# ishine/TTS-3

Measured on AMD Instinct MI355X. Metric: audio samples/sec + RTF, HiFiGAN-v1 22.05kHz 80-mel, batch 32 @ 1/2/4/8 GPU, higher is better.
Workload: dtype fp32 (power-of-2 scaled fp16 hi/lo split on fp16 MFMA, fp32 accumulate); 1 GPU; HiFiGAN-v1 22.05kHz inference, [32,80,1024] mel per GPU (replicate pad 5), fp32; model=HiFiGAN-v1 (hifigan_config.py generator_model_params), global_batch=32, seq_len=1024, parallelism=dp1 (utterance sharding; no collectives)

## Files before the change

tts-3_amd/csrc/common.hpp:

```cpp
#pragma once

#include <hip/hip_runtime.h>

#include <cstdint>
#include <stdexcept>
#include <string>

namespace tts {

struct Error : std::runtime_error {
  int code;
  Error(int c, const std::string& m) : std::runtime_error(m), code(c) {}
};

#define TTS_HIP_CHECK(expr)                                                               \
  do {                                                                                    \
    hipError_t _e = (expr);                                                               \
    if (_e != hipSuccess)                                                                 \
      throw ::tts::Error(2, std::string(#expr) + " failed: " + hipGetErrorString(_e));    \
  } while (0)

#define TTS_REQUIRE(cond, code, msg)                    \
  do {                                                  \
    if (!(cond)) throw ::tts::Error((code), (msg));     \
// ... 32 lines not shown
  int mask_res;
  int wn_rows;
  int gate;
  int planes;
};

constexpr int kSplitGateTile = 20;
constexpr int kSplitWinoTile = 21;
bool wino_supported(int mode, int Cout, int Cin, int K, int dil);
bool wino_enabled();
void launch_wino(int mode, const Conv1dArgs& a, int B, int K, hipStream_t s);
inline int gate_row_order(int rho, int H) {
  const int j = rho / 128, r = rho % 128;
  return r < 64 ? 64 * j + r : H + 64 * j + (r - 64);
}

struct ResPairArgs {
  Conv1dArgs c1;
  Conv1dArgs c2;
  const float* post_w;
  float post_bias;
  float post_slope;
  float* wav;
};
bool resblock_pair_supported(int mode, int C, int K, int dil);
bool resblock_pair_preferred(int mode, int C, int K, int dil);
bool resblock_pair128(int mode, int C, int K);
void launch_resblock_pair(int mode, const ResPairArgs& a, int B, int K, int C, int wide64, hipStream_t s);

struct ResBlock3Args {
  const float* x;
  const unsigned* amax_in;
  const float* w[6];
  const float* bias[6];
  int w_exp[6];
  int dil[3];
  float* z;
  int zmode;
  float zdiv;
  unsigned* amax_out;
  int T;
  int planes;
  const float* up_w;
  const float* up_bias;
  int up_w_exp;
  float* up_y;
  unsigned* up_amax;
  const float* zp[2];
  int nzp;
};
bool resblock3_supported(int mode, int C, int K, const int* dil);
bool resblock3_up_supported(int mode, int C, int K, const int* dil, int wide64);
constexpr int kWide64Block = 1, kWide64Pair = 2;
void launch_resblock3(int mode, const ResBlock3Args& a, int B, int C, int K, int wide64, hipStream_t s);
int mrf_geo64_wide(int mode);
bool resblock2_supported(int mode, int C, int K, const int* dil);
bool resblock2_preferred(int mode, int C, int K, const int* dil);
int resblock2_geo64(int mode);
void launch_resblock2(int mode, const ResBlock3Args& a, int B, int C, int K, int geo64, hipStream_t s);

struct ConvTile {
  int BM, BN, TM, TN, CK;
  int PD = 1;
  int WINO = 0;
};

struct ConvTArgs {
  const float* x;
  const float* w;
  const float* bias;
  float* y;
  int Cin, Cout, Tin;
  int n_chunks;
  float in_slope;
  unsigned* amax_out;
  const float* cvec;
};

struct PostArgs {
  const float* z;
  const float* w;
  float bias;
  float* y;
  int Cin, T;
  float in_slope;
  int z_b16;
};

int conv1d_tile_for(int Cout, int K, int Cin, int dil, bool res);
ConvTile conv1d_tile(int idx);
int conv1d_num_tiles();
void launch_conv1d(const Conv1dArgs& a, int B, int K, int tile_idx, hipStream_t s);
int convT_tile_for(int Cout, int U);
ConvTile convT_tile(int idx, int U);
void launch_convT(const ConvTArgs& a, int B, int U, int tile_idx, hipStream_t s);
void launch_conv_post(const PostArgs& a, int B, hipStream_t s);
void launch_mel_window(const float* mel, int B, int C, int T, int pad, int64_t w0, int W, float* out, hipStream_t s);
void launch_cond_vec(const float* g, const float* Wc, const float* bc, float* cvec, int B, int Cc,
                     int C0, hipStream_t s);

constexpr int MATH_FP32 = 0;
constexpr int MATH_FP32_X6 = 1;
constexpr int MATH_FP32_F16X3 = 2;
constexpr int MATH_BF16 = 3;
constexpr int MATH_LAST = MATH_BF16;

ConvTile conv1d_split_tile(int mode, int idx);
int conv1d_split_num_tiles(int mode);
// ... 45 lines not shown
```

tts-3_amd/csrc/hifigan.cpp:

```cpp
#include "hifigan.hpp"

#include <algorithm>
#include <cmath>
#include <cstdlib>
#include <vector>

namespace tts {

namespace {
bool valid_conv_k(int k) { return k == 1 || k == 3 || k == 5 || k == 7 || k == 11; }
}

std::vector<int64_t> hifigan_weight_shapes(const TtsHifiganCfg& c) {
  std::vector<int64_t> n;
  const int C0 = c.upsample_initial_channel;
  n.push_back((int64_t)C0 * c.in_channels * 7);
  n.push_back(C0);
  for (int i = 0; i < c.num_upsamples; ++i) {
    const int ci = C0 >> i, co = C0 >> (i + 1);
    n.push_back((int64_t)ci * co * c.upsample_kernel_sizes[i]);
    n.push_back(co);
  }
  for (int i = 0; i < c.num_upsamples; ++i) {
    const int ch = C0 >> (i + 1);
// ... 27 lines not shown
  TTS_REQUIRE(c.out_channels == 1, 3, "only out_channels == 1 is implemented");
  TTS_REQUIRE(c.resblock_type == 1 || c.resblock_type == 2, 1, "resblock_type must be '1' or '2'");
  TTS_REQUIRE(c.num_kernels >= 1 && c.num_kernels <= TTS_MAX_KERNELS, 1, "bad num_kernels");
  TTS_REQUIRE(c.num_upsamples >= 1 && c.num_upsamples <= TTS_MAX_UPSAMPLES, 1, "bad num_upsamples");
  const int need_d = c.resblock_type == 1 ? 3 : 2;
  TTS_REQUIRE(c.num_dilations >= need_d && c.num_dilations <= TTS_MAX_DILATIONS, 1,
              "resblock_dilation_sizes too short for the resblock type");
  for (int j = 0; j < c.num_kernels; ++j) {
    TTS_REQUIRE(valid_conv_k(c.resblock_kernel_sizes[j]), 3,
                "resblock kernel size " + std::to_string(c.resblock_kernel_sizes[j]) +
                    " not implemented (1,3,5,7,11)");
    for (int m = 0; m < need_d; ++m) {
      const int d = c.resblock_dilation_sizes[j][m];
      TTS_REQUIRE(d >= 1 && (c.resblock_kernel_sizes[j] - 1) * d <= 96, 3,
                  "resblock (kernel_size-1)*dilation must be <= 96");
    }
  }
  int C = c.upsample_initial_channel;
  for (int i = 0; i < c.num_upsamples; ++i) {
    const int u = c.upsample_factors[i];
    TTS_REQUIRE(u == 2 || u == 4 || u == 8, 3, "upsample factor must be 2, 4 or 8");
    TTS_REQUIRE(c.upsample_kernel_sizes[i] == 2 * u, 3,
                "upsample kernel size must equal 2*factor (polyphase kernel)");
    C >>= 1;
    TTS_REQUIRE(C >= 1, 1, "upsample_initial_channel too small for the number of upsamples");
  }
  TTS_REQUIRE(c.inference_padding >= 0, 1, "inference_padding must be >= 0");
  TTS_REQUIRE(c.cond_channels >= 0, 1, "cond_channels must be >= 0");
  TTS_REQUIRE(!c.cond_in_each_up_layer || c.cond_channels > 0, 1, "cond_in_each_up_layer needs cond_channels > 0");
  TTS_REQUIRE(c.math_mode >= MATH_FP32 && c.math_mode <= MATH_LAST, 1, "unknown math_mode");
}

Hifigan::Hifigan(const TtsHifiganCfg& cfg, const float* const* hw, int device)
    : cfg_(cfg), device_(device) {
  hifigan_validate(cfg_);
  DeviceGuard g(device_);
  const auto shapes = hifigan_weight_shapes(cfg_);
  for (size_t i = 0; i < shapes.size(); ++i)
    TTS_REQUIRE(hw[i] != nullptr, 1, "weight pointer " + std::to_string(i) + " is NULL");

  const int C0 = cfg_.upsample_initial_channel;
  const int mode = cfg_.math_mode;
  const char* nf = std::getenv("TTS_MI355X_NO_PAIR_FUSION");
  const bool pair_fusion = !(nf && nf[0] == '1');
  const char* pf = std::getenv("TTS_MI355X_POST_FUSION");
  post_fusion_ = !(pf && pf[0] == '0');
  const char* ms = std::getenv("TTS_MI355X_MRF_STREAMS");
  nbs_ = ms ? std::max(1, std::min(std::atoi(ms), cfg.num_kernels)) : cfg.num_kernels;
  nbs_env_ = ms != nullptr;
  const char* sb = std::getenv("TTS_MI355X_SUBBATCH");
  n_lanes_ = sb ? std::max(1, std::min(std::atoi(sb), 8)) : 2;
  rb2_geo64_ = resblock2_geo64(mode);
  geo64_wide_ = mrf_geo64_wide(mode);
  const char* bp = std::getenv("TTS_MI355X_BF16_PLANES");
  planes16_ = mode == MATH_BF16 && !(bp && bp[0] == '0') && cfg_.num_upsamples >= 1 &&
              cfg_.upsample_factors[0] % 8 == 0;
  size_t wi = 0;
  std::vector<std::pair<const float*, const float*>> src;
  auto add_conv = [&](int Cin, int Cout, int K, int dil, const char* fam, bool res, int lmode, bool pair128 = false) {
    ConvLayer L;
    L.Cin = Cin; L.Cout = Cout; L.K = K; L.dil = dil; L.pad = dil * (K - 1) / 2;
    L.mode = lmode;
    L.tile = conv_tile_for(lmode, Cout, K, Cin, dil, res);
    if (pair128) {
      L.tile = 7;
      L.name = std::string(fam) + "_k" + std::to_string(K) + "_c" + std::to_string(Cout);
      return L;
    }
    const bool wino_k3 = [] {
      const char* e = std::getenv("TTS_MI355X_WINO_K3");
      return e && e[0] == '1';
    }();
    const bool k_ok = K >= 7 || (K == 3 && Cout >= 256 && wino_k3);
    if (std::string(fam) == "mrf_conv" && k_ok && wino_enabled() && wino_supported(lmode, Cout, Cin, K, dil)) {
      L.tile = kSplitWinoTile;
      fam = "mrf_wino";
    }
    L.name = std::string(fam) + "_k" + std::to_string(K) + "_c" + std::to_string(Cout);
    return L;
  };

  pre_ = add_conv(cfg_.in_channels, C0, 7, 1, "conv_pre", false, mode);
  src.push_back({hw[wi], hw[wi + 1]}); wi += 2;
  for (int i = 0; i < cfg_.num_upsamples; ++i) {
    ConvTLayer L;
    L.Cin = C0 >> i; L.Cout = C0 >> (i + 1); L.U = cfg_.upsample_factors[i];
    L.mode = mode;
    L.tile = is_split_mode(mode) ? conv_tile_for(mode, L.U * L.Cout, 2, L.Cin, 1, false) : convT_tile_for(L.Cout, L.U);
    L.name = "ups_u" + std::to_string(L.U) + "_c" + std::to_string(L.Cout);
    ups_.push_back(L);
  }
  std::vector<std::pair<const float*, const float*>> usrc;
  for (int i = 0; i < cfg_.num_upsamples; ++i) { usrc.push_back({hw[wi], hw[wi + 1]}); wi += 2; }

  for (int i = 0; i < cfg_.num_upsamples; ++i) {
    const int ch = C0 >> (i + 1);
    for (int j = 0; j < cfg_.num_kernels; ++j) {
      const int k = cfg_.resblock_kernel_sizes[j];
      ResBlock rb;
      if (cfg_.resblock_type == 1) {
        const float* w1[3]; const float* b1[3]; const float* w2[3]; const float* b2[3];
        for (int m = 0; m < 3; ++m) { w1[m] = hw[wi]; b1[m] = hw[wi + 1]; wi += 2; }
        for (int m = 0; m < 3; ++m) { w2[m] = hw[wi]; b2[m] = hw[wi + 1]; wi += 2; }
        rb.fused = pair_fusion;
        const bool p128 = pair_fusion && resblock_pair128(mode, ch, k);
        bool tiles_ok = true;
        for (int m = 0; m < 3; ++m) {
          rb.convs.push_back(add_conv(ch, ch, k, cfg_.resblock_dilation_sizes[j][m], "mrf_conv", false, mode, p128));
          src.push_back({w1[m], b1[m]});
          rb.convs.push_back(add_conv(ch, ch, k, 1, "mrf_conv", true, mode, p128));
          src.push_back({w2[m], b2[m]});
          for (int c = 0; c < 2; ++c) {
            const ConvTile t = conv_tile(mode, rb.convs[2 * m + c].tile);
            const int dil = rb.convs[2 * m].dil;
            tiles_ok = tiles_ok && !t.WINO && t.CK % 16 == 0 && ch % t.CK == 0 && ch % t.BM == 0;
            rb.fused = rb.fused && !t.WINO && t.CK == 16 && ceil_div(ch, t.BM) * t.BM == ch &&
                       resblock_pair_preferred(mode, ch, k, dil);
          }
        }
        rb.fused3 = pair_fusion && tiles_ok;
      } else {
        bool tiles_ok = true;
        for (int m = 0; m < 2; ++m) {
          rb.convs.push_back(add_conv(ch, ch, k, cfg_.resblock_dilation_sizes[j][m], "mrf_conv", true, mode));
          src.push_back({hw[wi], hw[wi + 1]}); wi += 2;
          const ConvTile t = conv_tile(mode, rb.convs[m].tile);
          tiles_ok = tiles_ok && !t.WINO && t.CK % 16 == 0 && ch % t.CK == 0 && ch % t.BM == 0;
        }
        rb.fused2 = pair_fusion && tiles_ok;
      }
      if (rb.fused2 || (cfg_.resblock_type == 1 && rb.fused3)) {
        const int policy = [] {
          const char* e = std::getenv("TTS_MI355X_RESBLOCK3");
          if (!e) return 1 << 30;
          if (std::string(e) == "all") return 1 << 30;
          return std::atoi(e);
        }();
        const std::string wk = [] {
          const char* e = std::getenv("TTS_MI355X_RB1_WHOLE_K");
          return std::string(e ? e : "");
        }();
        const bool k_ok = k == 3 || wk.find(std::to_string(k)) != std::string::npos;
        if (cfg_.resblock_type == 1)
          rb.fused3 = ch <= policy && k_ok && resblock3_supported(mode, ch, k, cfg_.resblock_dilation_sizes[j]);
        else
          rb.fused2 = ch <= policy && resblock2_preferred(mode, ch, k, cfg_.resblock_dilation_sizes[j]);
      }
      res_.push_back(rb);
    }
  }
  ups_fused_.assign(cfg_.num_upsamples, 0);
  const char* uf = std::getenv("TTS_MI355X_UPS_FUSION");
  if (!(uf && uf[0] == '0') && cfg_.resblock_type == 1 && cfg_.num_kernels <= 3 && !cfg_.cond_in_each_up_layer &&
      !planes16_) {
    for (int i = 0; i + 1 < cfg_.num_upsamples; ++i) {
      const int ch = C0 >> (i + 1);
      const ConvTLayer& u = ups_[i + 1];
      if (!res_[i * cfg_.num_kernels].fused3 || u.U != 2 || !is_split_mode(u.mode)) continue;
      const ConvTile t = conv_tile(u.mode, u.tile);
      const bool tile_ok = !t.WINO && t.CK % 16 == 0 && ch % t.CK == 0 && ch % t.BM == 0;
      ups_fused_[i] = tile_ok && resblock3_up_supported(mode, ch, cfg_.resblock_kernel_sizes[0],
                                                        cfg_.resblock_dilation_sizes[0], geo64_wide_);
    }
  }
  const float* post_w = hw[wi]; wi += 1;
  post_bias_ = cfg_.conv_post_bias ? hw[wi][0] : 0.f;
  if (cfg_.conv_post_bias) wi += 1;

  HostArena arena;
  std::vector<ConvLayer*> convs;
  convs.push_back(&pre_);
  for (auto& rb : res_) for (auto& c : rb.convs) convs.push_back(&c);
  for (size_t i = 0; i < convs.size(); ++i) {
    ConvLayer& c = *convs[i];
    arena.put_conv(c, c.mode, conv_tile(c.mode, c.tile), src[i].first, src[i].second);
  }
  for (size_t i = 0; i < ups_.size(); ++i) {
    auto& u = ups_[i];
    if (is_split_mode(u.mode)) {
      const ConvTile t = conv_tile(u.mode, u.tile);
      u.n_chunks = ceil_div(u.Cin, t.CK);
      const size_t o = arena.alloc(packed_conv_numel(u.mode, u.U * u.Cout, u.Cin, 2, t), &u.w);
      u.w_exp = pack_convT_split(u.mode, usrc[i].first, u.Cin, u.Cout, u.U, t, arena.at(o));
      std::vector<float> bias((size_t)u.U * u.Cout);
      for (int co = 0; co < u.Cout; ++co)
        for (int ph = 0; ph < u.U; ++ph) bias[(size_t)co * u.U + ph] = usrc[i].second[co];
      arena.put_bias(bias.data(), u.U * u.Cout, t, &u.b);
    } else {
      const ConvTile t = convT_tile(u.tile, u.U);
      u.n_chunks = ceil_div(u.Cin, t.CK);
      const size_t o = arena.alloc(packed_convT_numel(u.Cin, u.Cout, u.U, t), &u.w);
      pack_convT(usrc[i].first, u.Cin, u.Cout, u.U, t, arena.at(o));
      arena.put_bias(usrc[i].second, u.Cout, t, &u.b);
    }
  }
// ... 333 lines not shown
      const hipStream_t sj = bj > 0 ? lane->branch[bj - 1] : s;
      float* bufX = ws + (2 + 2 * bj) * plane;
      float* bufT = bj == 0 ? bufT0 : bufX + plane;
      if (bj > 0) TTS_HIP_CHECK(hipStreamWaitEvent(sj, lane->ev_ups, 0));
      float* const xres = (fuse && j + 1 < K && (conc ? bstream(j + 1) : 0) == bj) ? bufZ : bufX;
      rplane[j] = xres;
      auto zorder = [&] {
        if (!fuse && bj > 0 && bstream(j - 1) != bj) TTS_HIP_CHECK(hipStreamWaitEvent(sj, lane->ev_z[j - 1], 0));
      };
      auto zdone = [&] {
        if (conc) TTS_HIP_CHECK(hipEventRecord(lane->ev_z[j], sj));
      };
      const int zlast = fuse ? 0 : ((cfg_.num_kernels == 1 || j == 0) ? 1 : (j == cfg_.num_kernels - 1 ? 3 : 2));
      const int gj = g0 + 1 + j * 6;
      const int gz = g0 + 1 + cfg_.num_kernels * 6;
      if (fuse && j == 0) {
        const ConvTLayer& Un = ups_[i + 1];
        ResBlock3Args ra{};
        ra.x = bufO; ra.amax_in = slots(g0);
        for (int c = 0; c < 6; ++c) { ra.w[c] = rb.convs[c].w; ra.bias[c] = rb.convs[c].b; ra.w_exp[c] = rb.convs[c].w_exp; }
        for (int m = 0; m < 3; ++m) ra.dil[m] = rb.convs[2 * m].dil;
        ra.zdiv = (float)K;
        ra.T = len;
        ra.nzp = K - 1;
        for (int p = 1; p < K; ++p) {
          ra.zp[p - 1] = rplane[p];
          if (conc && bstream(p) > 0) TTS_HIP_CHECK(hipStreamWaitEvent(s, lane->ev_z[p], 0));
        }
        ra.up_w = Un.w; ra.up_bias = Un.b; ra.up_w_exp = Un.w_exp;
        ra.up_y = bufT0; ra.up_amax = slots(stage_group(i + 1));
        const ConvLayer& L1 = rb.convs[0];
        const double flops = 12.0 * B * L1.Cout * (double)L1.Cin * L1.K * len +
                             2.0 * B * Un.Cout * (double)Un.Cin * 2 * (2.0 * len);
        const double bytes = 4.0 * B * L1.Cout * (double)len * (K + 1) + 4.0 * 6.0 * L1.Cout * L1.Cin * L1.K +
                             4.0 * Un.Cin * Un.Cout * 2 * Un.U;
        const std::string nm = "mrf_block_k" + std::to_string(L1.K) + "_c" + std::to_string(L1.Cout);
        run(prof, s, nm.c_str(), flops, bytes, [&] { launch_resblock3(L1.mode, ra, B, L1.Cout, L1.K, geo64_wide_, s); });
        std::swap(bufO, bufT0);
      } else if (cfg_.resblock_type == 1 && rb.fused3) {
        ResBlock3Args ra{};
        ra.x = bufO; ra.amax_in = slots(g0);
        ra.planes = planes16_ ? kPlaneXB16 | kPlaneYB16 : 0;
        for (int c = 0; c < 6; ++c) { ra.w[c] = rb.convs[c].w; ra.bias[c] = rb.convs[c].b; ra.w_exp[c] = rb.convs[c].w_exp; }
        for (int m = 0; m < 3; ++m) ra.dil[m] = rb.convs[2 * m].dil;
        ra.z = fuse ? xres : bufZ; ra.zmode = fuse ? 1 : zlast; ra.zdiv = (float)cfg_.num_kernels;
        ra.amax_out = !fuse && j == cfg_.num_kernels - 1 ? slots(gz) : nullptr;
        ra.T = len;
        const ConvLayer& L1 = rb.convs[0];
        const double flops = 12.0 * B * L1.Cout * (double)L1.Cin * L1.K * len;
        const double bytes = (planes16_ ? 2.0 : 4.0) * B * L1.Cout * len * (zlast >= 2 ? 3 : 2) +
                             4.0 * 6.0 * L1.Cout * L1.Cin * L1.K;
        const std::string nm = "mrf_block_k" + std::to_string(L1.K) + "_c" + std::to_string(L1.Cout);
        zorder();
        run(prof, sj, nm.c_str(), flops, bytes, [&] { launch_resblock3(L1.mode, ra, B, L1.Cout, L1.K, geo64_wide_, sj); });
        zdone();
      } else if (cfg_.resblock_type == 1 && rb.fused) {
        for (int m = 0; m < 3; ++m) {
          const ConvLayer& L1 = rb.convs[2 * m];
          const ConvLayer& L2 = rb.convs[2 * m + 1];
          const float* xin = (m == 0) ? bufO : (m == 1 ? bufX : bufT);
          const bool last = (m == 2);
          float* xout = (m == 1) ? bufT : (last ? xres : bufX);
          ResPairArgs pa{};
          Conv1dArgs& c1 = pa.c1;
          c1.x = xin; c1.w = L1.w; c1.bias = L1.b; c1.Cin = L1.Cin; c1.Cout = L1.Cout; c1.Tin = len; c1.Tout = len;
          c1.dil = L1.dil; c1.pad = L1.pad; c1.n_chunks = L1.n_chunks; c1.in_slope = 0.1f; c1.out_slope = 0.1f;
          c1.zdiv = 1.f; c1.w_exp = L1.w_exp;
          c1.planes = planes16_ ? kPlaneXB16 | kPlaneYB16 : 0;
          c1.amax_in = (m == 0) ? slots(g0) : slots(gj + 2 * m - 1);
          Conv1dArgs& c2 = pa.c2;
          c2.x = nullptr; c2.w = L2.w; c2.bias = L2.b; c2.res = xin; c2.y = xout; c2.z = bufZ;
          c2.Cin = L2.Cin; c2.Cout = L2.Cout; c2.Tin = len; c2.Tout = len; c2.dil = 1; c2.pad = L2.pad;
          c2.n_chunks = L2.n_chunks; c2.in_slope = 1.f; c2.out_slope = 1.f; c2.zmode = last ? zlast : 0;
          c2.zdiv = (float)cfg_.num_kernels; c2.w_exp = L2.w_exp;
          c2.planes = c1.planes;
          c2.amax_out = last ? (!fuse && j == cfg_.num_kernels - 1 ? slots(gz) : nullptr) : slots(gj + 2 * m + 1);
          const bool post = last && zlast == 3 && i == cfg_.num_upsamples - 1 && post_fusion_ &&
                            cfg_.out_channels == 1;
          if (post) {
            pa.post_w = post_wd_; pa.post_bias = post_bias_; pa.post_slope = 0.01f; pa.wav = wav;
            c2.amax_out = nullptr;
            post_done = true;
          }
          double flops = 4.0 * B * L1.Cout * (double)L1.Cin * L1.K * len;
          const double es = planes16_ ? 2.0 : 4.0;
          double bytes = es * B * L1.Cout * len * (last ? (zlast >= 2 ? 4 : 3) : 3) + 4.0 * 2.0 * L1.Cout * L1.Cin * L1.K;
          if (post) {
            flops += 2.0 * B * len * (double)L1.Cout * 7;
            bytes += 4.0 * B * len - es * B * L1.Cout * len;
          }
          const std::string nm = std::string(post ? "mrf_pair_post_k" : "mrf_pair_k") + std::to_string(L1.K) +
                                 "_c" + std::to_string(L1.Cout);
          if (last) zorder();
          run(prof, sj, nm.c_str(), flops, bytes, [&] { launch_resblock_pair(L1.mode, pa, B, L1.K, L1.Cout, geo64_wide_, sj); });
          if (last) zdone();
        }
      } else if (cfg_.resblock_type == 1) {
        for (int m = 0; m < 3; ++m) {
          const float* xin = (m == 0) ? bufO : bufX;
          const unsigned* xin_amax = (m == 0) ? slots(g0) : slots(gj + 2 * m - 1);
          const bool last = (m == 2);
          conv(rb.convs[2 * m], xin, len, len, 0, 0.1f, 0.1f, nullptr, bufT, 0, nullptr, xin_amax, slots(gj + 2 * m),
               sj);
          if (last) zorder();
          conv(rb.convs[2 * m + 1], bufT, len, len, 0, 1.f, 1.f, xin, last ? xres : bufX, last ? zlast : 0, nullptr,
               slots(gj + 2 * m), last ? (!fuse && j == cfg_.num_kernels - 1 ? slots(gz) : nullptr) : slots(gj + 2 * m + 1), sj);
          if (last) zdone();
// ... 47 lines not shown
```

tts-3_amd/csrc/hifigan.hpp:

```cpp
#pragma once

#include <string>
#include <vector>

#include "arena.hpp"
#include "common.hpp"
#include "tts_mi355x.h"

namespace tts {

struct Profiler {
  struct Rec {
    std::string name;
    double flops, bytes;
    hipEvent_t a, b;
  };
  std::vector<Rec> recs;
  ~Profiler() {
    for (auto& r : recs) {
      (void)hipEventDestroy(r.a);
      (void)hipEventDestroy(r.b);
    }
  }
};
// ... 28 lines not shown
  void reserve(int B, int T, int pad);
  void forward(const float* mel, int B, int C, int T, int pad, const float* g, float* wav,
               hipStream_t s, Profiler* prof);
  int device() const { return device_; }
  int window_halo() const;
  int64_t max_window_frames() const;
  int64_t window_payload() const;

 private:
  struct ConvLayer : PackedConv {
    int mode = 0;
    std::string name;
  };
  struct ConvTLayer : PackedConv {
    int U = 0;
    int mode = 0;
    std::string name;
  };
  struct ResBlock {
    std::vector<ConvLayer> convs;
    bool fused = false;
    bool fused3 = false;
    bool fused2 = false;
  };

  struct Lane {
    hipStream_t own = nullptr;
    std::vector<hipStream_t> branch;
    hipEvent_t ev_ups = nullptr, ev_done = nullptr;
    std::vector<hipEvent_t> ev_z;
    int nbs = 1;
  };
  void forward_plain(const float* mel, int B, int C, int T, int pad, const float* g, float* wav, hipStream_t s,
                     Profiler* prof, float* ws, Lane* lane);
  void ensure_lanes();
  int64_t lane_bytes(int B, int64_t L, int nbs) const;
  int lane_batch(int B, int i) const { return B / n_lanes_ + (i < B % n_lanes_ ? 1 : 0); }
  bool windowed(int64_t L) const;
  int64_t plain_workspace_bytes(int B, int64_t L, bool window) const;
  int64_t window_buffer_bytes(int B, int64_t W) const;
  void reserve_plain(int B, int64_t L, bool window = false);
  int64_t plane_floats(int B, int T, int pad) const;
  int64_t cond_floats(int B) const;
  int amax_groups() const;
  int stage_group(int i) const;
  int n_planes(int nbs) const;
  int split_nbs() const;

  TtsHifiganCfg cfg_;
  int device_;
  int hop_ = 1;
  int rb2_geo64_ = 0;
  int geo64_wide_ = 0;
  bool post_fusion_ = true;
  bool planes16_ = false;
  std::vector<char> ups_fused_;
  int nbs_ = 1;
  int n_lanes_ = 2;
  bool nbs_env_ = false;
  std::vector<Lane> lanes_;
  hipEvent_t ev_start_ = nullptr;
  ConvLayer pre_;
  std::vector<ConvTLayer> ups_;
  std::vector<ResBlock> res_;
  float post_bias_ = 0.f;
  float* post_wd_ = nullptr;
  float* cond_wd_ = nullptr;
  float* cond_bd_ = nullptr;
  std::vector<std::pair<float*, float*>> up_cond_;
  DeviceBuffer arena_, ws_;
  DeviceBuffer win_;
};

}
```

tts-3_amd/csrc/kernels_resblock.hip:

```cpp
#include <algorithm>
#include <cstdlib>
#include <type_traits>

#include "resblock_block.hpp"
#include "split_device.hpp"

namespace tts {




constexpr int kPostK = 7;
constexpr int kPostHalo = 3;

template <class S, int K, int C, int PD, int GEO, bool ALLX = false, bool POST = false, bool SWZ = false>
struct PairCfg {
  static_assert(!SWZ || (GEO == 0 && C == 64 && S::NP == 2 && ALLX), "SWZ: GEO 0 at 64 channels, two-piece rows");
  using ROWS = Res3Rows<S::NP, SWZ>;
  static constexpr int PITCH = ROWS::PITCH;
  static_assert(SWZ || PITCH == S::ROWB, "the padded layout is the scheme's own row");
  static constexpr int RP_W = (GEO == 0 || GEO == 4 || GEO == 5 || GEO == 7) ? 256 : (GEO == 1 ? 192 : 128);
  static constexpr int LEAD = (K - 1) / 2;
  static constexpr int RP_BN = RP_W - 2 * LEAD;
  static constexpr int NW = GEO >= 5 ? 8 : 4;
// ... 461 lines not shown
  const char* e256 = std::getenv("TTS_MI355X_PAIR256");
  if (C == 128) return (K == 7 || K == 11) && !(e128 && e128[0] == '0');
  if (C == 256) {
    const char* e11 = std::getenv("TTS_MI355X_PAIR256_K11");
    return (K == 3 || K == 7 || (K == 11 && e11 && e11[0] == '1')) && !(e256 && e256[0] == '0');
  }
  return false;
}

bool resblock_pair_preferred(int mode, int C, int K, int dil) {
  return resblock_pair_supported(mode, C, K, dil);
}

void launch_resblock_pair(int mode, const ResPairArgs& a, int B, int K, int C, int wide64, hipStream_t s) {
  TTS_REQUIRE(resblock_pair_supported(mode, C, K, a.c1.dil), 3, "resblock pair: unsupported configuration");
  TTS_REQUIRE(a.c1.Cin == C && a.c1.Cout == C && a.c2.Cin == C && a.c2.Cout == C && a.c1.Tin == a.c1.Tout &&
                  a.c2.Tout == a.c1.Tout && a.c1.rep_pad == 0 && a.c2.dil == 1,
              1, "resblock pair: bad arguments");
  TTS_REQUIRE(a.c2.res != a.c2.y || a.c2.zmode != 0, 1, "resblock pair: x and x' must not alias");
  TTS_REQUIRE(a.c1.cvec == nullptr && a.c2.cvec == nullptr && a.c1.bias && a.c2.bias, 1,
              "resblock pair: biases required, no cond vector (both are staged in LDS)");
  TTS_REQUIRE((int64_t)C * a.c1.Tout * 4 < (int64_t(1) << 31), 3, "resblock pair: plane exceeds 2 GiB");
  TTS_REQUIRE(!a.post_w || (a.c2.zmode == 3 && a.c2.res && a.c2.z && a.wav && !a.c2.mask), 1,
              "resblock pair: the fused conv_post needs the final MRF sum (zmode 3) with a residual");
  if (mode == MATH_FP32_F16X3) launch_pair_s<SchemeH3>(a, B, K, C, wide64, s);
  else if (mode == MATH_BF16) launch_pair_s<SchemeB1>(a, B, K, C, 0, s);
  else launch_pair_s<SchemeX6>(a, B, K, C, 0, s);
  TTS_HIP_CHECK(hipGetLastError());
}


namespace {
template <class S, int C, int GEO, int K>
void launch_res3_t(const ResBlock3Args& a, int B, hipStream_t s) {
  using P = Res3Cfg<S, C, GEO, K, 6, r3_xoff(K), r3_lead(K)>;
  dim3 grid(ceil_div(a.T, P::RP_BN), 1, B);
  launch_block_pl<S, C, GEO, K, 6, r3_xoff(K), r3_lead(K)>(a, grid, P::NT, s);
}
template <class S, int C, int GEO>
void launch_res3_up_t(const ResBlock3Args& a, int B, hipStream_t s) {
  using P = Res3Cfg<S, C, GEO, 3, 6, r3_xoff(3), r3_lead(3), true>;
  dim3 grid(ceil_div(a.T, P::RP_BN), 1, B);
  hipLaunchKernelGGL((resblock3_kernel<S, C, GEO, 3, 6, r3_xoff(3), r3_lead(3), 0, true>), grid, dim3(P::NT), 0, s, a);
}
template <class S, bool UP>
void launch_res3_wide64(const ResBlock3Args& a, int B, hipStream_t s) {
  using P = Res3Cfg<S, 64, 0, 3, 6, r3_xoff(3), r3_lead(3), UP, true>;
  static_assert(P::RP_BN == 232, "kept columns [12, 244)");
  dim3 grid(ceil_div(a.T, P::RP_BN), 1, B);
  hipLaunchKernelGGL((resblock3_kernel<S, 64, 0, 3, 6, r3_xoff(3), r3_lead(3), 0, UP, true>), grid, dim3(P::NT), 0, s, a);
}
template <class S>
void launch_res3_s(const ResBlock3Args& a, int B, int C, int K, int wide64, hipStream_t s) {
  if (K == 7) {
    if (C == 32) launch_res3_t<S, 32, 0, 7>(a, B, s);
    else launch_res3_t<S, 64, 0, 7>(a, B, s);
    return;
  }
  if (K == 11) {
    if (C == 32) launch_res3_t<S, 32, 0, 11>(a, B, s);
    else launch_res3_t<S, 64, 0, 11>(a, B, s);
    return;
  }
  if constexpr (std::is_same<S, SchemeH3>::value) {
    if (C == 64 && (wide64 & kWide64Block) && a.planes == 0) {
      launch_res3_wide64<S, false>(a, B, s);
      return;
    }
  }
  if (C == 32) launch_res3_t<S, 32, 0, 3>(a, B, s);
  else if (C == 128) {
    if constexpr (S::NP == 2) launch_res3_t<S, 128, 4, 3>(a, B, s);
    else if constexpr (S::ROWB <= 80) launch_res3_t<S, 128, 3, 3>(a, B, s);
    else throw Error(3, "resblock3: 128 channels need a split scheme of at most 80-byte rows");
  } else launch_res3_t<S, 64, 2, 3>(a, B, s);
}
}

bool resblock3_supported(int mode, int C, int K, const int* dil) {
  if (!is_split_mode(mode)) return false;
  if (K == 3) {
    if (!(C == 32 || C == 64 || (C == 128 && mode != MATH_FP32_X6))) return false;
  } else if (K == 7 || K == 11) {
    if (!(C == 32 || C == 64)) return false;
  } else {
    return false;
  }
  const int hk = (K - 1) / 2;
  int lo = -r3_xoff(K);
  for (int m = 0; m < 3; ++m) {
    if (dil[m] < 1 || hk * dil[m] > r3_xoff(K)) return false;
    lo = std::max(lo + hk * dil[m], 0) + hk;
  }
  return lo <= r3_lead(K);
}

int mrf_geo64_wide(int mode) {
  if (mode != MATH_FP32_F16X3) return 0;
  const char* e = std::getenv("TTS_MI355X_GEO64_WIDE");
  return e && e[0] == '0' ? 0 : (kWide64Block | kWide64Pair);
}

bool resblock3_up_supported(int mode, int C, int K, const int* dil, int wide64) {
  if (mode != MATH_FP32_F16X3 || K != 3 || !(C == 64 || C == 128) || !resblock3_supported(mode, C, K, dil)) return false;
  const int rp_w = C == 64 && (wide64 & kWide64Block) ? 256 : 128;
  int lo = -r3_xoff(K), hi = rp_w + r3_xoff(K);
  for (int m = 0; m < 3; ++m) {
    lo = std::max(lo + dil[m], 0) + 1;
    hi = std::min(hi - dil[m], rp_w) - 1;
  }
  return lo <= r3_lead(K) - 1 && hi >= rp_w - r3_lead(K) + 1;
}

void launch_resblock3(int mode, const ResBlock3Args& a, int B, int C, int K, int wide64, hipStream_t s) {
  TTS_REQUIRE(resblock3_supported(mode, C, K, a.dil), 3, "resblock3: unsupported configuration");
  TTS_REQUIRE((int64_t)C * a.T * 4 < (int64_t(1) << 31), 3, "resblock3: plane exceeds 2 GiB");
  if (a.up_w) {
    TTS_REQUIRE(resblock3_up_supported(mode, C, K, a.dil, wide64), 3, "resblock3: no upsampling tail for this configuration");
    TTS_REQUIRE(a.x && a.up_y && a.up_y != a.x && a.up_bias && a.planes == 0 && a.nzp >= 0 && a.nzp <= 2, 1,
                "resblock3: bad arguments of the upsampling tail");
    for (int p = 0; p < a.nzp; ++p)
      TTS_REQUIRE(a.zp[p] && a.zp[p] != a.up_y, 1, "resblock3: a branch plane is missing or aliases the tail's output");
    if (C == 128) launch_res3_up_t<SchemeH3, 128, 4>(a, B, s);
    else if (wide64 & kWide64Block) launch_res3_wide64<SchemeH3, true>(a, B, s);
    else launch_res3_up_t<SchemeH3, 64, 2>(a, B, s);
    TTS_HIP_CHECK(hipGetLastError());
    return;
  }
  TTS_REQUIRE(a.zmode >= 1 && a.zmode <= 3 && a.z && a.x && a.x != a.z, 1, "resblock3: bad arguments");
  if (mode == MATH_FP32_F16X3) launch_res3_s<SchemeH3>(a, B, C, K, wide64, s);
  else if (mode == MATH_BF16) launch_res3_s<SchemeB1>(a, B, C, K, 0, s);
  else launch_res3_s<SchemeX6>(a, B, C, K, 0, s);
  TTS_HIP_CHECK(hipGetLastError());
}

bool resblock2_supported(int mode, int C, int K, const int* dil) {
  if (!is_split_mode(mode) || !(K == 3 || K == 5 || K == 7 || K == 11)) return false;
  if (!(C == 32 || C == 64 || (C == 128 && mode != MATH_FP32_X6 && (K == 3 || K == 5)))) return false;
  const int H = rb2_halo(K), hk = (K - 1) / 2;
  int lo = -H;
  for (int m = 0; m < 2; ++m) {
    if (dil[m] < 1 || hk * dil[m] > H) return false;
    lo = std::max(lo + hk * dil[m], 0);
  }
  return lo <= H;
}

bool resblock2_preferred(int mode, int C, int K, const int* dil) {
  if (!resblock2_supported(mode, C, K, dil)) return false;
  const char* e = std::getenv("TTS_MI355X_RB2_ALL");
  if (e && e[0] == '1') return true;
  return mode == MATH_BF16 || !(C == 64 && K == 11);
}
// ... 19 lines not shown
```

tts-3_amd/csrc/resblock_block.hpp:

```cpp
#pragma once
#include <type_traits>

#include "res3_layout.hpp"
#include "split_device.hpp"

#ifndef RES_PD_B1
#define RES_PD_B1 2
#endif
#ifndef RES_STAGE_8R
#define RES_STAGE_8R 1
#endif

namespace tts {

#ifndef R3_XR_POL
#define R3_XR_POL 0
#endif
constexpr int R3_XOFF = 5;
constexpr int R3_LEAD = 12;
constexpr int r3_xoff(int K) { return R3_XOFF * ((K - 1) / 2); }
constexpr int r3_lead(int K) { return R3_LEAD * ((K - 1) / 2); }
constexpr int rb2_halo(int K) { return K == 3 ? 4 : (K == 5 ? 12 : (K == 7 ? 9 : 15)); }

template <class S, int C, int GEO, int K = 3, int NCV = 6, int XO = R3_XOFF, int LEAD = R3_LEAD, bool UP = false,
          bool SW = false>
struct Res3Cfg {
  static_assert(!SW || (GEO == 0 && S::NP == 2), "SW: GEO 0's tile, two-piece rows");
  static constexpr bool SWZ = (GEO == 4 || SW) && S::NP == 2;
  static constexpr bool W64 = GEO == 4 || SW;
  static constexpr int RP_W = GEO == 0 ? 256 : (GEO == 1 ? 192 : 128);
  static constexpr int RP_BN = RP_W - 2 * LEAD;
  static constexpr int NW = GEO == 3 ? 8 : 4;
  static constexpr int NT = 64 * NW;
  static constexpr int WN = GEO == 0 ? 4 : 2;
  static constexpr int WM = NW / WN;
  static constexpr int TM = C / 32 / WM;
  static constexpr int TN = RP_W / 32 / WN;
  static constexpr int NC = C / 16;
  static constexpr int PR = RP_W + 2 * XO;
  using ROWS = Res3Rows<S::NP, SWZ>;
  static_assert(SWZ || ROWS::PITCH == S::ROWB, "the padded layout is the scheme's own row");
  static constexpr int LDSB = NC * PR * ROWS::PITCH;
  static constexpr int LDS_TOTAL = LDSB + 2 * NW * 4 + (NCV + UP) * C * 4;
  static_assert(!W64 || LDS_TOTAL <= 80 * 1024, "GEO 4 / SW: two workgroups per CU");
  static_assert(TM >= 1 && TM * WM * 32 == C && TN * WN * 32 == RP_W, "geometry");
};

#ifndef RB3_W_B1
#define RB3_W_B1 0
#endif
#ifndef RB3_W64
#define RB3_W64 2
#endif
template <class S, int C, int GEO, int K, int NCV, int XO, int LEAD, int PL = 0, bool UP = false, bool SW = false>
__global__ __launch_bounds__((Res3Cfg<S, C, GEO, K, NCV, XO, LEAD>::NT))
__attribute__((amdgpu_waves_per_eu(S::NP == 1 && RB3_W_B1 > 0 ? RB3_W_B1
                                                                : (C == 64 && GEO == 2 ? RB3_W64 : (C == 32 || GEO >= 3 || SW ? 2 : 1)))))
void resblock3_kernel(ResBlock3Args a) {
  constexpr bool XB = (PL & kPlaneXB16) != 0, YB = (PL & kPlaneYB16) != 0;
  using PX = PlaneT<XB>;
  using PY = PlaneT<YB>;
  using P = Res3Cfg<S, C, GEO, K, NCV, XO, LEAD, UP, SW>;
  using ROWS = typename P::ROWS;
  static_assert(NCV == 6 || NCV == 2, "ResBlock1 (6 convs) or ResBlock2 (2 convs)");
  static_assert(!UP || (NCV == 6 && S::SCALED && PL == 0), "the upsampling tail: ResBlock1, f16x3, fp32 planes");
  constexpr int NP = S::NP;
  constexpr bool H3 = S::SCALED;
  constexpr int TM = P::TM, TN = P::TN, NC = P::NC, PR = P::PR, RP_W = P::RP_W;
  constexpr int PD = S::NP == 1 ? RES_PD_B1 : 2;
  __shared__ __attribute__((aligned(16))) unsigned char smem[P::LDSB];
  constexpr int NT = P::NT;
  __shared__ float red[2][P::NW];
  __shared__ float bsm[(NCV + UP) * C];

  const int tid = threadIdx.x;
  const int lane = tid & 63;
  const int wave = tid >> 6;
  const int half = lane >> 5;
  const int l32 = lane & 31;
  const int wm = __builtin_amdgcn_readfirstlane(wave / P::WN);
  const int wn = wave % P::WN;
  const int mrow0 = wm * TM * 32;
  const int t0 = blockIdx.x * P::RP_BN;
  const int b = blockIdx.z;
  const int T = a.T;
  const int tx0 = t0 - LEAD;
  const int xcol0 = wn * TN * 32 + l32;
  const unsigned avoff = (unsigned)lane * 16u;
  const unsigned chb = (unsigned)T * PX::ES;
  const rsrc_t rx = make_rsrc(plane_at<XB>(a.x, (size_t)b * C * T), (unsigned)C * chb);
  auto ldx = [&](unsigned off, auto pol_tag, unsigned soff = 0u) -> float {
    if constexpr (XB) return PX::ld(rx, off, soff);
    else return bload_x<decltype(pol_tag)::value>(rx, off, soff);
  };
  constexpr bool SOFF = P::W64;

  int ex = H3 ? amax_exp(a.amax_in, b) : 0;
  f32x16 xr[TM][TN];
// ... 493 lines not shown
```

Measured before the change: 171.4 million samples/s.

## Add wide 512-column GEO 5 tile for 32-channel fused ResBlock1 with K=7/11

Adds a new Res3Cfg geometry (GEO 5) for 32-channel ResBlock1: 512-column tiles, 4 waves laid out along time, swizzled two-piece LDS rows, sized so two workgroups fit per CU. It also enables the whole-block fused path for the K=7 resblock at 32 channels, which previously ran unfused unless an env var listed K=7. The wider tile cuts halo recompute per kept column and the fusion cuts global traffic between convs, at the cost of more LDS per workgroup and possibly fewer blocks in flight. A host-side test replays LDS addressing to check for bank conflicts.

```diff
diff --git a/tts-3_amd/csrc/common.hpp b/tts-3_amd/csrc/common.hpp
--- a/tts-3_amd/csrc/common.hpp
+++ b/tts-3_amd/csrc/common.hpp
@@ -108,8 +108,10 @@
 bool resblock3_supported(int mode, int C, int K, const int* dil);
 bool resblock3_up_supported(int mode, int C, int K, const int* dil, int wide64);
 constexpr int kWide64Block = 1, kWide64Pair = 2;
+constexpr int kWide32Block = 4;
 void launch_resblock3(int mode, const ResBlock3Args& a, int B, int C, int K, int wide64, hipStream_t s);
 int mrf_geo64_wide(int mode);
+int mrf_geo32_wide(int mode);
 bool resblock2_supported(int mode, int C, int K, const int* dil);
 bool resblock2_preferred(int mode, int C, int K, const int* dil);
 int resblock2_geo64(int mode);
diff --git a/tts-3_amd/csrc/hifigan.cpp b/tts-3_amd/csrc/hifigan.cpp
--- a/tts-3_amd/csrc/hifigan.cpp
+++ b/tts-3_amd/csrc/hifigan.cpp
@@ -103,6 +103,7 @@
   n_lanes_ = sb ? std::max(1, std::min(std::atoi(sb), 8)) : 2;
   rb2_geo64_ = resblock2_geo64(mode);
   geo64_wide_ = mrf_geo64_wide(mode);
+  geo32_wide_ = mrf_geo32_wide(mode);
   const char* bp = std::getenv("TTS_MI355X_BF16_PLANES");
   planes16_ = mode == MATH_BF16 && !(bp && bp[0] == '0') && cfg_.num_upsamples >= 1 &&
               cfg_.upsample_factors[0] % 8 == 0;
@@ -191,7 +192,8 @@
           const char* e = std::getenv("TTS_MI355X_RB1_WHOLE_K");
           return std::string(e ? e : "");
         }();
-        const bool k_ok = k == 3 || wk.find(std::to_string(k)) != std::string::npos;
+        const bool k7_block = k == 7 && ch == 32 && (geo32_wide_ & kWide32Block) != 0 && j + 1 < cfg_.num_kernels;
+        const bool k_ok = k == 3 || k7_block || wk.find(std::to_string(k)) != std::string::npos;
         if (cfg_.resblock_type == 1)
           rb.fused3 = ch <= policy && k_ok && resblock3_supported(mode, ch, k, cfg_.resblock_dilation_sizes[j]);
         else
@@ -631,7 +633,8 @@
                              4.0 * 6.0 * L1.Cout * L1.Cin * L1.K;
         const std::string nm = "mrf_block_k" + std::to_string(L1.K) + "_c" + std::to_string(L1.Cout);
         zorder();
-        run(prof, sj, nm.c_str(), flops, bytes, [&] { launch_resblock3(L1.mode, ra, B, L1.Cout, L1.K, geo64_wide_, sj); });
+        run(prof, sj, nm.c_str(), flops, bytes,
+            [&] { launch_resblock3(L1.mode, ra, B, L1.Cout, L1.K, geo64_wide_ | geo32_wide_, sj); });
         zdone();
       } else if (cfg_.resblock_type == 1 && rb.fused) {
         for (int m = 0; m < 3; ++m) {
diff --git a/tts-3_amd/csrc/hifigan.hpp b/tts-3_amd/csrc/hifigan.hpp
--- a/tts-3_amd/csrc/hifigan.hpp
+++ b/tts-3_amd/csrc/hifigan.hpp
@@ -104,6 +104,7 @@
   int hop_ = 1;
   int rb2_geo64_ = 0;
   int geo64_wide_ = 0;
+  int geo32_wide_ = 0;
   bool post_fusion_ = true;
   bool planes16_ = false;
   std::vector<char> ups_fused_;
diff --git a/tts-3_amd/csrc/kernels_resblock.hip b/tts-3_amd/csrc/kernels_resblock.hip
--- a/tts-3_amd/csrc/kernels_resblock.hip
+++ b/tts-3_amd/csrc/kernels_resblock.hip
@@ -537,6 +537,13 @@
 }
 template <class S>
 void launch_res3_s(const ResBlock3Args& a, int B, int C, int K, int wide64, hipStream_t s) {
+  if constexpr (std::is_same<S, SchemeH3>::value) {
+    if (C == 32 && (K == 7 || K == 11) && (wide64 & kWide32Block) && a.planes == 0) {
+      if (K == 7) launch_res3_t<S, 32, 5, 7>(a, B, s);
+      else launch_res3_t<S, 32, 5, 11>(a, B, s);
+      return;
+    }
+  }
   if (K == 7) {
     if (C == 32) launch_res3_t<S, 32, 0, 7>(a, B, s);
     else launch_res3_t<S, 64, 0, 7>(a, B, s);
@@ -584,6 +591,12 @@
   if (mode != MATH_FP32_F16X3) return 0;
   const char* e = std::getenv("TTS_MI355X_GEO64_WIDE");
   return e && e[0] == '0' ? 0 : (kWide64Block | kWide64Pair);
+}
+
+int mrf_geo32_wide(int mode) {
+  if (mode != MATH_FP32_F16X3) return 0;
+  const char* e = std::getenv("TTS_MI355X_GEO32_WIDE");
+  return e && e[0] == '0' ? 0 : kWide32Block;
 }
 
 bool resblock3_up_supported(int mode, int C, int K, const int* dil, int wide64) {
diff --git a/tts-3_amd/csrc/resblock_block.hpp b/tts-3_amd/csrc/resblock_block.hpp
--- a/tts-3_amd/csrc/resblock_block.hpp
+++ b/tts-3_amd/csrc/resblock_block.hpp
@@ -44,6 +44,28 @@
   static constexpr int LDS_TOTAL = LDSB + 2 * NW * 4 + (NCV + UP) * C * 4;
   static_assert(!W64 || LDS_TOTAL <= 80 * 1024, "GEO 4 / SW: two workgroups per CU");
   static_assert(TM >= 1 && TM * WM * 32 == C && TN * WN * 32 == RP_W, "geometry");
+};
+
+template <class S, int C, int K, int NCV, int XO, int LEAD, bool UP, bool SW>
+struct Res3Cfg<S, C, 5, K, NCV, XO, LEAD, UP, SW> {
+  static_assert(C == 32 && S::NP == 2 && NCV == 6 && !UP && !SW, "GEO 5: the 32-channel ResBlock1, two-piece rows");
+  static constexpr bool SWZ = true;
+  static constexpr bool W64 = true;
+  static constexpr int RP_W = 512;
+  static constexpr int RP_BN = RP_W - 2 * LEAD;
+  static constexpr int NW = 4;
+  static constexpr int NT = 64 * NW;
+  static constexpr int WN = 4;
+  static constexpr int WM = 1;
+  static constexpr int TM = 1;
+  static constexpr int TN = RP_W / 32 / WN;
+  static constexpr int NC = C / 16;
+  static constexpr int PR = RP_W + 2 * XO;
+  using ROWS = Res3Rows<S::NP, SWZ>;
+  static constexpr int LDSB = NC * PR * ROWS::PITCH;
+  static constexpr int LDS_TOTAL = LDSB + 2 * NW * 4 + NCV * C * 4;
+  static_assert(LDS_TOTAL <= 80 * 1024, "GEO 5: two workgroups per CU");
+  static_assert(RP_BN > 0 && TN * WN * 32 == RP_W, "geometry");
 };
 
 #ifndef RB3_W_B1
diff --git a/tts-3_amd/tests_native/geo32_layout_check.cpp b/tts-3_amd/tests_native/geo32_layout_check.cpp
--- /dev/null
+++ b/tts-3_amd/tests_native/geo32_layout_check.cpp
@@ -0,0 +1,178 @@
+#include <algorithm>
+#include <cstdio>
+#include <vector>
+
+#include "common.hpp"
+#include "res3_layout.hpp"
+
+using namespace tts;
+
+static int failures = 0;
+#define CHECK(cond, ...)                          \
+  do {                                            \
+    if (!(cond)) {                                \
+      if (failures < 20) {                        \
+        std::fprintf(stderr, "FAIL: " __VA_ARGS__); \
+        std::fprintf(stderr, "\n");               \
+      }                                           \
+      ++failures;                                 \
+    }                                             \
+  } while (0)
+
+using R = Res3Rows<2, true>;
+constexpr int NP = 2, NC = 2, RP_W = 512, NT = 256, TN = 4, C = 32, NCV = 6, PITCH = R::PITCH;
+static long n_reads = 0, n_stores = 0;
+
+static int worst(const std::vector<int>& addr, const std::vector<int>& lanes, int dw, int banks) {
+  std::vector<std::vector<int>> on(banks);
+  for (int l : lanes) {
+    if (addr[l] < 0) continue;
+    for (int j = 0; j < dw; ++j) {
+      const int d = addr[l] / 4 + j;
+      auto& v = on[d % banks];
+      if (std::find(v.begin(), v.end(), d) == v.end()) v.push_back(d);
+    }
+  }
+  size_t w = 0;
+  for (const auto& v : on) w = std::max(w, v.size());
+  return (int)w;
+}
+
+static std::vector<std::vector<int>> read128_groups() {
+  const int a[2][16] = {{0, 1, 2, 3, 12, 13, 14, 15, 20, 21, 22, 23, 24, 25, 26, 27},
+                        {4, 5, 6, 7, 8, 9, 10, 11, 16, 17, 18, 19, 28, 29, 30, 31}};
+  std::vector<std::vector<int>> g;
+  for (int h = 0; h < 2; ++h)
+    for (int s = 0; s < 2; ++s) {
+      std::vector<int> v;
+      for (int i = 0; i < 16; ++i) v.push_back(a[s][i] + 32 * h);
+      g.push_back(v);
+    }
+  return g;
+}
+static std::vector<std::vector<int>> contiguous_groups(int n) {
+  std::vector<std::vector<int>> g;
+  for (int l0 = 0; l0 < 64; l0 += n) {
+    std::vector<int> v;
+    for (int i = 0; i < n; ++i) v.push_back(l0 + i);
+    g.push_back(v);
+  }
+  return g;
+}
+
+static const std::vector<std::vector<int>> RG = read128_groups(), W8 = contiguous_groups(8), W16 = contiguous_groups(16);
+
+static void expect_read(const std::vector<int>& addr, const char* what, int a, int b, int c, int d) {
+  for (const auto& grp : RG)
+    CHECK(worst(addr, grp, 4, 64) == 1, "%s: ds_read_b128 conflict (%d %d %d %d)", what, a, b, c, d);
+  ++n_reads;
+}
+static void expect_store(const std::vector<int>& addr, bool b128, const char* what, int a, int b, int c, int d) {
+  for (const auto& grp : b128 ? W8 : W16)
+    CHECK(worst(addr, grp, b128 ? 4 : 2, 32) <= 2, "%s: %s conflict above 2-way (%d %d %d %d)", what,
+          b128 ? "ds_write_b128" : "ds_write_b64", a, b, c, d);
+  ++n_stores;
+}
+
+static void check_block(int K) {
+  const int HK = (K - 1) / 2, XO = 5 * HK, LEAD = 12 * HK, PR = RP_W + 2 * XO, LDSB = NC * PR * PITCH;
+  CHECK(LDSB == 2 * (512 + 2 * XO) * 64, "k%d: LDS region %d B", K, LDSB);
+  CHECK(LDSB + 2 * 4 * 4 + NCV * C * 4 <= 80 * 1024, "k%d: LDS %d B does not fit twice", K, LDSB);
+  CHECK(RP_W - 2 * LEAD == (K == 3 ? 488 : (K == 7 ? 440 : 392)), "k%d: kept columns", K);
+  std::vector<int> addr(64);
+  struct Tap { int roff, kstep; };
+  std::vector<Tap> taps;
+  for (int d : {1, 3, 5}) taps.push_back({XO - HK * d, d});
+  taps.push_back({0, 1});
+  for (const Tap& t : taps) {
+    CHECK(t.roff >= 0 && t.roff + (K - 1) * t.kstep <= 2 * XO, "k%d: tap offsets leave the staged rows", K);
+    CHECK(t.kstep == 1 || (t.roff - XO == -HK * t.kstep && HK * t.kstep <= 25), "k%d: offsets up to +-25", K);
+    for (int g = 0; g < NC; ++g)
+      for (int wn = 0; wn < 4; ++wn)
+        for (int n = 0; n < TN; ++n)
+          for (int k = 0; k < K; ++k)
+            for (int q = 0; q < NP; ++q) {
+              for (int lane = 0; lane < 64; ++lane) {
+                const int half = lane >> 5, row = g * PR + wn * TN * 32 + (lane & 31) + t.roff + k * t.kstep;
+                addr[lane] = R::piece(R::off(row, half), q) + n * 32 * PITCH;
+                CHECK(row + n * 32 >= g * PR && row + n * 32 < (g + 1) * PR, "k%d: read row outside group %d", K, g);
+                CHECK(addr[lane] >= 0 && addr[lane] + 16 <= LDSB, "k%d: read leaves the LDS array", K);
+                CHECK(addr[lane] == R::off(row + n * 32, half + 2 * q), "k%d: read unit map, row %d", K, row + n * 32);
+              }
+              expect_read(addr, "block tap", K, t.roff, t.kstep, k);
+            }
+  }
+  for (int roff : {XO, HK}) {
+    for (int g = 0; g < NC; ++g)
+      for (int wn = 0; wn < 4; ++wn)
+        for (int n = 0; n < TN; ++n)
+          for (int p = 0; p < NP; ++p) {
+            for (int lane = 0; lane < 64; ++lane) {
+              const int half = lane >> 5, row = g * PR + wn * TN * 32 + (lane & 31) + roff;
+              addr[lane] = R::piece(R::off(row, half), p) + n * 32 * PITCH;
+              CHECK(row + n * 32 >= g * PR + roff && row + n * 32 < g * PR + roff + RP_W, "k%d: store_pieces row", K);
+              CHECK(addr[lane] == R::off(row + n * 32, half + 2 * p), "k%d: store_pieces unit map", K);
+              CHECK(addr[lane] >= 0 && addr[lane] + 16 <= LDSB, "k%d: store_pieces leaves the LDS array", K);
+            }
+            expect_store(addr, true, "block store_pieces", K, roff, g, wn * TN + n);
+          }
+    const int EB = 2 * XO * PITCH, lead_b = roff * PITCH, tail_b = (PR - roff - RP_W) * PITCH;
+    std::vector<int> zeroed(LDSB / 16, 0);
+    for (int e0 = 0; e0 < NC * EB; e0 += NT * 16)
+      for (int wave = 0; wave < 4; ++wave) {
+        for (int lane = 0; lane < 64; ++lane) {
+          const int e = e0 + (wave * 64 + lane) * 16;
+          addr[lane] = -1;
+          if (e >= NC * EB) continue;
+          const int g = e / EB, o = e - g * EB;
+          if (o < lead_b) addr[lane] = g * PR * PITCH + o;
+          else if (o - lead_b < tail_b) addr[lane] = (g * PR + roff + RP_W) * PITCH + (o - lead_b);
+          if (addr[lane] >= 0) {
+            CHECK(addr[lane] + 16 <= LDSB, "k%d: edge zeroing leaves the LDS array", K);
+            ++zeroed[addr[lane] / 16];
+          }
+        }
+        expect_store(addr, true, "block edge rows", K, roff, e0, wave);
+      }
+    for (int g = 0; g < NC; ++g)
+      for (int r = 0; r < PR; ++r)
+        for (int u = 0; u < 4; ++u) {
+          const bool edge = r < roff || r >= roff + RP_W;
+          CHECK(zeroed[((g * PR + r) * PITCH + 16 * u) / 16] == (edge ? 1 : 0), "k%d: edge zeroing of row %d (roff %d)", K, r, roff);
+        }
+  }
+  std::vector<int> staged(LDSB / 8, 0);
+  for (int g = 0; g < NC; ++g)
+    for (int u0 = 0; u0 < ((PR * 4 + NT - 1) / NT) * NT; u0 += 64)
+      for (int p = 0; p < NP; ++p) {
+        for (int lane = 0; lane < 64; ++lane) {
+          const int u = u0 + lane;
+          const int q = quad_pos((u >> 3) & 3), r = (u >> 5) * 8 + (u & 7), qp = quad_pos(q);
+          addr[lane] = r < PR ? R::off(g * PR + r, (qp >> 1) + 2 * p) + 8 * (qp & 1) : -1;
+          if (addr[lane] >= 0) {
+            CHECK(addr[lane] >= (g * PR + r) * PITCH && addr[lane] + 8 <= (g * PR + r + 1) * PITCH,
+                  "k%d: prologue store leaves row %d of group %d", K, r, g);
+            ++staged[addr[lane] / 8];
+          }
+        }
+        expect_store(addr, false, "block prologue", K, g, u0, p);
+      }
+  for (int s : staged) CHECK(s == 1, "k%d: the prologue stages an 8-byte slot %d times", K, s);
+}
+
+int main() {
+  static_assert(R::PITCH == 64 && R::SWIZZLED, "the swizzled two-piece row");
+  for (int K : {3, 7, 11}) check_block(K);
+  {
+    std::vector<int> addr(64);
+    for (int lane = 0; lane < 64; ++lane) addr[lane] = (lane & 31) * 64 + 16 * (lane >> 5);
+    CHECK(worst(addr, RG[0], 4, 64) == 4, "the replay does not see the 4-way conflict of plain 64-byte rows");
+  }
+  if (failures) {
+    std::fprintf(stderr, "%d layout check(s) failed\n", failures);
+    return 1;
+  }
+  std::printf("geo32_layout_check: %ld read and %ld store instructions replayed: reads conflict-free, stores at most 2-way\n",
+              n_reads, n_stores);
+  return 0;
+}
```

Result: faster. 173.8 million samples/s, median of 6 (+1.4%).
